# OpenBMB/VisRAG

Hardware: AMD Instinct MI355X
Metric: page-images embedded/sec (VisRAG-Ret encode, 448x448, bf16 MFMA) + queries/sec@top-10 over 100k-page index (higher is better)
Workload: dtype bf16; 1 GPU; VisRAG-Ret (SigLIP-so400m 26 blk + resampler + MiniCPM-2B 40 layers) bf16 encode batch=32 page images 448x448 per GPU; index 100000 rows x 2304 sharded 1 way(s), 1000 queries top-10; batch_per_gpu=32, global_batch=32, parallelism=dp1 (pages sharded, no data-path collective)

## Files before the change

include/visrag_hip.h:

```cpp
#ifndef VISRAG_HIP_H
#define VISRAG_HIP_H

#include <stddef.h>
#include <stdint.h>

#ifdef __cplusplus
extern "C" {
#endif

#define VR_OK 0
#define VR_ERR_INVALID 1
#define VR_ERR_HIP 2
#define VR_ERR_STATE 3
#define VR_ERR_CAPACITY 4

#define VR_DTYPE_F32 0
#define VR_DTYPE_BF16 1

typedef struct vr_model_s* vr_model_t;
typedef struct vr_index_s* vr_index_t;

typedef struct vr_config {
    int32_t patch_size;
    int32_t vit_dim;
// ... 172 lines not shown

int vr_op_gemm(int device_id, const void* A, int32_t lda, const void* W, int32_t ldw,
               int32_t M, int32_t N, int32_t K, int32_t epilogue, const float* bias,
               const float* resid, float alpha, void* out, int32_t ldo,
               const int32_t* rope_pos, const float* rope_table, int32_t rope_cols,
               int32_t variant, void* stream);
typedef struct vr_gemm_extras {
    const int32_t* rowmap;
    const float* rowbias;
    int32_t rowbias_period, rowbias_ld, rowbias_cols;
    float col_scale;
    int32_t col_scale_n;
    int32_t ksplit;
    int64_t split_stride;
    const int32_t* m_dev;
    int32_t m_sub;
    int32_t raster_gm;
} vr_gemm_extras_t;
int vr_op_gemm_ex(int device_id, const void* A, int32_t lda, const void* W, int32_t ldw,
                  int32_t M, int32_t N, int32_t K, int32_t epilogue, const float* bias,
                  const float* resid, float alpha, void* out, int32_t ldo,
                  const int32_t* rope_pos, const float* rope_table, int32_t rope_cols,
                  int32_t variant, const vr_gemm_extras_t* extras, void* stream);
int vr_op_norm(int device_id, int32_t kind, const float* x, int32_t rows, int32_t dim,
               const float* weight, const float* bias, float eps, void* out, int32_t ldo,
               void* stream);
int vr_op_norm_ex(int device_id, int32_t kind, const float* x, int32_t rows, int32_t dim, int32_t ldx, const float* weight,
                  const float* bias, float eps, void* out, int32_t ldo, void* stream);

int vr_op_text_rmsnorm_split(int device_id, const float* x, int32_t rows, int32_t dim, const float* weight, float eps, void* hi,
                             void* lo, void* stream);
int vr_op_text_rope(int device_id, float* qkv, int32_t T, int32_t ld, int32_t rope_cols, const int32_t* pos, const float* table,
                    void* stream);
int vr_op_text_attention(int device_id, const float* qkv, int32_t ld, int32_t E, const int32_t* seq_offsets, int32_t B, int32_t T,
                         int32_t heads, float scale, float* out, void* stream);
int vr_op_text_swiglu_split(int device_id, const float* gu, int32_t T, int32_t ld_gu, int32_t I, int32_t ld_act, void* hi, void* lo,
                            void* stream);
int vr_op_embed_gather(int device_id, const int32_t* ids, int32_t T, const void* table, const void* table_lo, int32_t dim,
                       float scale, float* out, void* stream);
int vr_op_pool(int device_id, const float* h, const int32_t* seq_offsets, int32_t B, int32_t dim, const float* norm_w, float eps,
               float* out, float* tap, int32_t mode, void* stream);
int vr_op_convert(int device_id, int32_t kind, const void* in, void* out, void* out2, int64_t n, int64_t n_total, int32_t* aux,
                  void* stream);
int vr_op_planes_sum(int device_id, const float* parts, int32_t n_parts, int64_t stride, int32_t ldp, int32_t T, int32_t N,
                     float* out, int32_t ldo, float alpha, int32_t accumulate, void* stream);
int vr_op_patch_embed(int device_id, const void* const* imgs, int32_t n, int32_t H, int32_t W, int32_t P, const float* weight,
// ... 45 lines not shown
```

visrag_amd/_lib.py:

```python
from __future__ import annotations

import ctypes as C
import os
from typing import Optional

_HERE = os.path.dirname(os.path.abspath(__file__))
LIB_PATH = os.path.join(_HERE, "libvisrag_hip.so")

VR_DTYPE_F32, VR_DTYPE_BF16 = 0, 1


class VRConfig(C.Structure):
    _fields_ = [
        ("patch_size", C.c_int32), ("vit_dim", C.c_int32), ("vit_depth", C.c_int32),
        ("vit_heads", C.c_int32), ("vit_hidden", C.c_int32), ("vit_pos_grid", C.c_int32),
        ("vit_ln_eps", C.c_float), ("query_num", C.c_int32), ("resampler_ln_eps", C.c_float),
        ("hidden_size", C.c_int32), ("num_layers", C.c_int32), ("num_heads", C.c_int32),
        ("intermediate_size", C.c_int32), ("vocab_size", C.c_int32), ("rms_norm_eps", C.c_float),
        ("rope_theta", C.c_float), ("scale_emb", C.c_float), ("residual_scale", C.c_float),
        ("max_images", C.c_int32), ("max_patches", C.c_int32), ("max_tokens", C.c_int32),
        ("max_seqs", C.c_int32), ("text_split_precision", C.c_int32),
    ]


# ... 73 lines not shown
    "vr_index_search_keys": (C.c_int, [_vp, _vp, _i32, _i32, _i64, _vp, _i32, _vp]),
    "vr_index_set_groups": (C.c_int, [_vp, C.POINTER(_i64), _i64]),
    "vr_index_search_groups": (C.c_int, [_vp, _vp, _i32, _i32, _vp, _vp, _vp, _i32, _vp]),
    "vr_index_group_search_stats": (C.c_int, [_vp, C.POINTER(_i64), _i32]),
    "vr_index_set_filters": (C.c_int, [_vp, _vp, _i32, _i32, _vp]),
    "vr_index_search_filtered": (C.c_int, [_vp, _vp, _i32, _i32, _vp, _vp, _vp, _i32, _vp]),
    "vr_index_filter_search_stats": (C.c_int, [_vp, C.POINTER(_i64), _i32]),
    "vr_index_search_range": (C.c_int, [_vp, _vp, _i32, _vp, _vp, _i64, _vp, C.POINTER(_i64), _i32, _vp]),
    "vr_index_range_results": (C.c_int, [_vp, _vp, _vp, _i64, _i32, _vp]),
    "vr_index_range_search_stats": (C.c_int, [_vp, C.POINTER(_i64), _i32]),
    "vr_index_rank_rows": (C.c_int, [_vp, _vp, _i32, _vp, _vp, _vp, _vp, _vp, _i32, _vp]),
    "vr_index_count_range": (C.c_int, [_vp, _vp, _i32, _vp, _vp, _i32, _vp, _vp, _i32, _vp]),
    "vr_index_rank_search_stats": (C.c_int, [_vp, C.POINTER(_i64), _i32]),
    "vr_index_search_diverse": (C.c_int, [_vp, _vp, _i32, _i32, _i32, _f32, _vp, _vp, _vp, _i32, _vp]),
    "vr_index_remove": (C.c_int, [_vp, C.POINTER(_i64), _i64, C.POINTER(_i64), _vp]),
    "vr_index_update": (C.c_int, [_vp, C.POINTER(_i64), _vp, _i64, _i32, _vp]),
    "vr_index_get_rows": (C.c_int, [_vp, C.POINTER(_i64), _i64, _vp, _vp, _i32, _vp]),
    "vr_topk_merge_keys": (C.c_int, [C.c_int, _vp, _i32, _i32, _i32, _vp, _vp, _vp]),
    "vr_resize_bicubic": (C.c_int, [C.c_int, _vp, _i32, _i32, _i32, _vp, _i32, _i32, _vp]),
    "vr_op_gemm": (C.c_int, [C.c_int, _vp, _i32, _vp, _i32, _i32, _i32, _i32, _i32, _vp, _vp, _f32,
                             _vp, _i32, _vp, _vp, _i32, _i32, _vp]),
    "vr_op_gemm_ex": (C.c_int, [C.c_int, _vp, _i32, _vp, _i32, _i32, _i32, _i32, _i32, _vp, _vp, _f32,
                                _vp, _i32, _vp, _vp, _i32, _i32, C.POINTER(VRGemmExtras), _vp]),
    "vr_op_norm": (C.c_int, [C.c_int, _i32, _vp, _i32, _i32, _vp, _vp, _f32, _vp, _i32, _vp]),
    "vr_op_norm_ex": (C.c_int, [C.c_int, _i32, _vp, _i32, _i32, _i32, _vp, _vp, _f32, _vp, _i32, _vp]),
    "vr_op_text_rmsnorm_split": (C.c_int, [C.c_int, _vp, _i32, _i32, _vp, _f32, _vp, _vp, _vp]),
    "vr_op_text_rope": (C.c_int, [C.c_int, _vp, _i32, _i32, _i32, _vp, _vp, _vp]),
    "vr_op_text_attention": (C.c_int, [C.c_int, _vp, _i32, _i32, _vp, _i32, _i32, _i32, _f32, _vp, _vp]),
    "vr_op_text_swiglu_split": (C.c_int, [C.c_int, _vp, _i32, _i32, _i32, _i32, _vp, _vp, _vp]),
    "vr_op_embed_gather": (C.c_int, [C.c_int, _vp, _i32, _vp, _vp, _i32, _f32, _vp, _vp]),
    "vr_op_pool": (C.c_int, [C.c_int, _vp, _vp, _i32, _i32, _vp, _f32, _vp, _vp, _i32, _vp]),
    "vr_op_convert": (C.c_int, [C.c_int, _i32, _vp, _vp, _vp, _i64, _i64, _vp, _vp]),
    "vr_op_planes_sum": (C.c_int, [C.c_int, _vp, _i32, _i64, _i32, _i32, _i32, _vp, _i32, _f32, _i32, _vp]),
    "vr_op_patch_embed": (C.c_int, [C.c_int, C.POINTER(_vp), _i32, _i32, _i32, _i32, _vp, _i32, _i32, _vp, _vp, _i32, _vp, _i32, _vp]),
    "vr_op_attention": (C.c_int, [C.c_int, _vp, _i32, _vp, _i32, _vp, _i32, _vp, _i32, _vp, _vp, _i32,
                                  _i32, _i32, _i32, _i32, _i32, _f32, _vp]),
    "vr_op_attention_ex": (C.c_int, [C.c_int, _vp, _i32, _vp, _i32, _vp, _i32, _vp, _i32, _vp, _vp, _i32,
                                     _i32, _i32, _i32, _i32, _i32, _f32, C.POINTER(VRAttnExtras), _vp]),
    "vr_op_attn_combine": (C.c_int, [C.c_int, _vp, _vp, _i32, _vp, _i32, _i32, _i32, _vp, _i32, _vp, _i32, _i32, _i32, _i32, _i32,
                                     _i32, _i32, _i64, _vp]),
    "vr_op_gemm_skinny": (C.c_int, [C.c_int, _vp, _i32, _vp, _i32, _i32, _i32, _i32, _i32, _vp, _i32, _vp, _i32, _i64, _vp]),
    "vr_op_plane_sum": (C.c_int, [C.c_int, _i32, _vp, _i32, _i64, _i32, _i32, _i32, _vp, _i32, _f32, _vp, _f32, _vp, _i32, _vp]),
    "vr_op_chat_attention": (C.c_int, [C.c_int, _vp, _vp, _vp, _i32, _i32, _i32, _i32, _i32, _i32, _i32, _i32, C.POINTER(_i32),
                                       C.POINTER(_i32), C.POINTER(_i32), C.POINTER(_i32), _i32, _vp, _vp]),
    "vr_op_chat_select": (C.c_int, [C.c_int, _i32, _vp, _i32, _i32, _vp, _i32, _i32, C.POINTER(_i32), C.POINTER(_f32), _i32, _i32,
                                    _f32, _f32, C.c_uint64, _i32, C.POINTER(_f32), C.POINTER(_i32), C.POINTER(_i32), _vp]),
# ... 77 lines not shown
```

visrag_amd/csrc/encode.hip:

```cpp
#include <hip/hip_runtime.h>

#include <algorithm>
#include <cmath>
#include <cstring>
#include <vector>

#include "model.h"

static int run_vision_group(vr_model_s* m, const uint8_t* const* dev_imgs_hostarray, int n, int H, int W,
                            const int32_t* rowmap_host , bool first_group, hipStream_t s) {
    const vr_config_t& c = m->c;
    const int P = c.patch_size, gh = H / P, gw = W / P, N = gh * gw;
    const int D = m->D, Dp = m->Dp, E = m->E, Q = m->Q;
    const int M = n * N;
    GridTables* g = nullptr;
    VRCHK(get_grid(m, gh, gw, &g));

    HIPCHK(hipMemcpyAsync(m->w_imgptr.p, dev_imgs_hostarray, (size_t)n * 8, hipMemcpyHostToDevice, s));
    int* cu = (int*)arena_take(m, (size_t)2 * (n + 1) * 4);
    for (int i = 0; i <= n; ++i) { cu[i] = i * N; cu[n + 1 + i] = i * Q; }
    HIPCHK(hipMemcpyAsync(m->w_cu.p, cu, (size_t)2 * (n + 1) * 4, hipMemcpyHostToDevice, s));
    HIPCHK(hipMemcpyAsync(m->w_rowmap.p, rowmap_host, (size_t)n * Q * 4, hipMemcpyHostToDevice, s));
    const int* cu_tok = m->w_cu.as<int>();
    const int* cu_qry = m->w_cu.as<int>() + (n + 1);
// ... 335 lines not shown
        }
        if (ks > 1) {
            GemmArgs a = gemm_args(A, lda, L, T, part, E);
            a.ksplit = ks; a.split_stride = pstride;
            HIPCHK(launch_gemm(a, EPI_F32, gemm256w_fits(a, route.proj_variant == GEMM_VARIANT_192W ? 192 : 256) ? route.proj_variant : GEMM_VARIANT_256IL, s));
            pend = true;
        } else {
            GemmArgs a = gemm_args(A, lda, L, T, h, E); a.resid = h; a.alpha = c.residual_scale;
            HIPCHK(launch_gemm(a, EPI_RESID, GEMM_VARIANT_AUTO, s));
        }
        return VR_OK;
    };
    auto norm = [&](const float* w) -> int {
        VRCHK(prof_begin(m, VR_PROF_DEC_NORM, s));
        struct End { vr_model_s* m; hipStream_t s; ~End() { (void)prof_end(m, VR_PROF_DEC_NORM, 0.0, s); } } end_{m, s};
        if (pend) {
            HIPCHK(launch_rmsnorm_accum(h, T, E, E, part, ks, pstride, E, c.residual_scale, w, c.rms_norm_eps, m->w_dxn.p, E, s));
            pend = false;
        } else {
            HIPCHK(launch_rmsnorm(h, T, E, E, w, c.rms_norm_eps, m->w_dxn.p, E, s));
        }
        return VR_OK;
    };
    double attn_flops = 0;
    for (int i = 0; i < B; ++i) { const double Li = seq_offsets[i + 1] - seq_offsets[i]; attn_flops += 4.0 * Li * Li * E; }
    for (int l = 0; l < c.num_layers; ++l) {
        const DecLayer& L = m->layers[l];
        VRCHK(norm(L.ln1.v.as<float>()));
        {
            GemmArgs a = gemm_args(m->w_dxn.p, E, L.qkv, T, m->w_dqkv.p, 3 * E);
            a.rope_pos = m->w_pos.as<int>(); a.rope_table = m->rope.as<float>(); a.rope_cols = 2 * E;
            VRCHK(prof_begin(m, VR_PROF_DEC_QKV, s));
            HIPCHK(launch_gemm(a, EPI_ROPE, GEMM_VARIANT_AUTO, s));
            VRCHK(prof_end(m, VR_PROF_DEC_QKV, 6.0 * T * (double)E * E, s));
        }
        if (hook && hook->layer) VRCHK(hook->layer(hook->ctx, l, m->w_dqkv.p, 3 * E, T, s));
        {
            VRCHK(prof_begin(m, VR_PROF_DEC_ATTN, s));
            AttnArgs a{};
            a.q = m->w_dqkv.p; a.ldq = 3 * E; a.k = (const char*)m->w_dqkv.p + (size_t)E * 2; a.ldk = 3 * E;
            a.v = (const char*)m->w_dqkv.p + (size_t)2 * E * 2; a.ldv = 3 * E;
            a.out = m->w_datt.p; a.ldo = E; a.cu_q = seq; a.cu_kv = seq; a.B = B; a.heads = c.num_heads; a.head_dim = 64;
            a.max_q = max_len; a.causal = 1; a.q_shared = 0; a.scale = 1.0f / sqrtf(64.0f);
            HIPCHK(launch_attention(a, s));
            VRCHK(prof_end(m, VR_PROF_DEC_ATTN, attn_flops, s));
        }
        VRCHK(prof_begin(m, VR_PROF_DEC_O, s));
        VRCHK(proj(m->w_datt.p, E, L.o));
        VRCHK(prof_end(m, VR_PROF_DEC_O, 2.0 * T * (double)E * E, s));
        VRCHK(norm(L.ln2.v.as<float>()));
        VRCHK(prof_begin(m, VR_PROF_DEC_GU, s));
        {
            GemmArgs a = gemm_args(m->w_dxn.p, E, L.gu, T, m->w_dact.p, m->Ip);
            HIPCHK(launch_gemm(a, EPI_SWIGLU, GEMM_VARIANT_AUTO, s));
        }
        VRCHK(prof_end(m, VR_PROF_DEC_GU, 4.0 * T * (double)E * m->I, s));
        VRCHK(prof_begin(m, VR_PROF_DEC_DOWN, s));
        VRCHK(proj(m->w_dact.p, m->Ip, L.down));
        VRCHK(prof_end(m, VR_PROF_DEC_DOWN, 2.0 * T * (double)E * m->I, s));
        if (l == 0) VRCHK(tap_store(m, "dec_layer0", h, T, E, E, false, s));
    }
    if (pend) {
        HIPCHK(launch_rmsnorm_accum(h, T, E, E, part, ks, pstride, E, c.residual_scale, nullptr, c.rms_norm_eps, nullptr, 0, s));
        pend = false;
    }
    }
    {
        double fl = 0;
        for (int i = 0; i < B; ++i) { const double Li = seq_offsets[i + 1] - seq_offsets[i]; fl += 4.0 * Li * Li * E; }
        fl = c.num_layers * (fl + (double)T * (8.0 * E * E + 6.0 * (double)E * m->I));
        VRCHK(prof_end(m, VR_PROF_DECODER, fl, s));
    }
    float* tap_hidden = nullptr;
    if (m->taps_on && (size_t)T * E * 4 <= m->w_kv32.bytes) tap_hidden = m->w_kv32.as<float>();
    if (out_hidden) {
        if (max_len > hidden_len) return fail(VR_ERR_INVALID, "hidden_len=%d is shorter than the longest sequence (%d)", hidden_len, max_len);
// ... 19 lines not shown
```

visrag_amd/csrc/gemm.hip:

```cpp
#include "gemm_core.h"
#include "gemm_core_il.h"
#include "kernels.h"
#include "gemm_epilogue.h"

namespace vr {

template <int EPI>
__global__ __launch_bounds__(256) void gemm_bf16_kernel(GemmArgs p) {
    extern __shared__ __attribute__((aligned(16))) char smem[];
    const int tiles_n = p.N / GEMM_BN;
    const int tiles_m = (p.M + GEMM_BM - 1) / GEMM_BM;
    const int t = xcd_remap(blockIdx.x, tiles_m * tiles_n);
    const int GM = p.raster_gm > 0 ? p.raster_gm : 1;
    const int gsz = GM * tiles_n;
    const int g = t / gsz, r = t % gsz;
    const int gm = min(GM, tiles_m - g * GM);
    const int m0 = (g * GM + r % gm) * GEMM_BM, n0 = (r / gm) * GEMM_BN;

    gemm_acc_t acc;
    gemm_zero(acc);
    gemm_mainloop(acc, (const bf16_t*)p.A, p.lda, (const bf16_t*)p.W, p.ldw, m0, n0, p.K, smem);

    const int lane = threadIdx.x & 63, wave = threadIdx.x >> 6;
    const int wm = wave >> 1, wn = wave & 1;
// ... 78 lines not shown
        return hipGetLastError();
    }
    if (variant != GEMM_VARIANT_GLDS) return hipErrorInvalidValue;
    const int tiles = (a.N / GEMM_BN) * ((a.M + GEMM_BM - 1) / GEMM_BM);
    if (a.raster_gm <= 0) {
        const int tm = (a.M + GEMM_BM - 1) / GEMM_BM;
        a.raster_gm = tm <= 32 ? tm : 4;
    }
    auto k = gemm_bf16_kernel<EPI>;
    static unsigned long long attr = 0;
    set_max_dynamic_lds((const void*)k, GEMM_SMEM_BYTES, attr);
    hipLaunchKernelGGL(k, dim3(tiles), dim3(256), GEMM_SMEM_BYTES, s, a);
    return hipGetLastError();
}

bool gemm_args_refused(const GemmArgs& a, int epi, int variant) {
    if (a.col_scale_n != 0 && (epi != EPI_BF16 || a.col_scale_n < 0 || a.col_scale_n % 64 != 0)) return true;
    const bool half_tile = variant == GEMM_VARIANT_128W_192 || variant == GEMM_VARIANT_128W_256;
    const bool split_tile = variant == GEMM_VARIANT_256IL || variant == GEMM_VARIANT_256W || variant == GEMM_VARIANT_192W;
    if (half_tile && (a.rowmap || a.rowbias)) return true;
    if (a.rowbias && ((epi != EPI_BF16 && epi != EPI_GELU && epi != EPI_F32) || a.rowbias_period < 1)) return true;
    if (a.ksplit > 1 && (!split_tile || epi != EPI_F32 || a.K % (a.ksplit * GEMM_BK) || a.rowmap || a.rowbias)) return true;
    if (a.m_dev && variant != GEMM_VARIANT_256IL) return true;
    return false;
}

hipError_t launch_gemm(const GemmArgs& a, int epi, int variant, hipStream_t s) {
    if (a.M <= 0) return hipSuccess;
    if (variant == GEMM_VARIANT_192) return launch_gemm192(a, epi, s);
    if (variant == GEMM_VARIANT_256W) return launch_gemm256w(a, epi, s);
    if (variant == GEMM_VARIANT_192W) return launch_gemm192w(a, epi, s);
    if (variant == GEMM_VARIANT_128W_192) return launch_gemm128w(a, epi, 192, s);
    if (variant == GEMM_VARIANT_128W_256) return launch_gemm128w(a, epi, 256, s);
    if (variant == GEMM_VARIANT_AUTO) {
        if (a.N % 192 == 0 && a.N % 256 != 0 && a.N <= 1536 && a.M >= 4096 && epi <= EPI_RESID) {
            if (epi == EPI_RESID && !a.rowmap && gemm256w_fits(a, 192)) return launch_gemm192w(a, epi, s);
            return launch_gemm192(a, epi, s);
        }
        const bool n_ok = (a.N % 256 == 0) || a.N >= 2048;
        const long t256 = (long)((a.N + 255) / 256) * ((a.M + 255) / 256);
        const long t128 = (long)(a.N / 128) * ((a.M + 127) / 128);
        const double e256 = 1.45 * (double)t256 / (double)(((t256 + 255) / 256) * 256);
        const double e128 = (double)t128 / (double)(((t128 + 511) / 512) * 512);
        const bool w_ok = gemm256w_fits(a, 256);
        variant = (n_ok && e256 > e128) ? (w_ok ? GEMM_VARIANT_256W : GEMM_VARIANT_256IL) : GEMM_VARIANT_GLDS;
        if (variant == GEMM_VARIANT_256W) return launch_gemm256w(a, epi, s);
    }
    if (gemm_args_refused(a, epi, variant)) return hipErrorInvalidValue;
    switch (epi) {
        case EPI_BF16: return launch_epi<EPI_BF16>(a, variant, s);
        case EPI_GELU: return launch_epi<EPI_GELU>(a, variant, s);
        case EPI_F32: return launch_epi<EPI_F32>(a, variant, s);
        case EPI_RESID: return launch_epi<EPI_RESID>(a, variant, s);
        case EPI_SWIGLU: return launch_epi<EPI_SWIGLU>(a, variant, s);
        case EPI_ROPE: return launch_epi<EPI_ROPE>(a, variant, s);
        default: return hipErrorInvalidValue;
    }
}

}
```

visrag_amd/csrc/gemm256w.hip:

```cpp
#include <type_traits>

#include "gemm_core.h"
#include "gemm_epilogue.h"
#include "gemm256w_acc.h"

namespace vr {

bool gemm256w_fits(const GemmArgs& a, int bn);

namespace {

constexpr int W_STAGE = 2 * G256_TILE_BYTES;
constexpr unsigned W_OOB = 0x80000000u;

}

constexpr int W_STAGING = 4096;
constexpr int W_SMEM_BYTES = 2 * W_STAGE + 4 * W_STAGING;

#define W_KERNEL_TEMPLATE template <int EPI, bool PLAIN, int NJ>
#define W_KERNEL_NAME gemm256w_bf16_kernel
#include "gemm256w_kernel.h"
#undef W_KERNEL_TEMPLATE
#undef W_KERNEL_NAME

template <int EPI, bool PLAIN, int NJ>
static hipError_t launch_wp(GemmArgs a, hipStream_t s) {
    constexpr int BN = 32 * NJ;
    const int tn = (a.N + BN - 1) / BN, tm = (a.M + G256_BM - 1) / G256_BM;
    if (a.raster_gm <= 0) a.raster_gm = tm <= 16 ? tm : 4;
    if (!gemm256w_fits(a, BN)) return hipErrorInvalidValue;
    if (gemm_args_refused(a, EPI, NJ == 6 ? GEMM_VARIANT_192W : GEMM_VARIANT_256W)) return hipErrorInvalidValue;
    int total = tn * tm;
    if (a.ksplit > 1) total *= a.ksplit;
    auto k = gemm256w_bf16_kernel<EPI, PLAIN, NJ>;
    static unsigned long long attr = 0;
    set_max_dynamic_lds((const void*)k, W_SMEM_BYTES, attr);
    hipLaunchKernelGGL(k, dim3(total), dim3(256), W_SMEM_BYTES, s, a);
    return hipGetLastError();
}

// ... 37 lines not shown
```

visrag_amd/csrc/gemm256w_kernel.h:

```cpp
W_KERNEL_TEMPLATE
__global__ __launch_bounds__(256) __attribute__((amdgpu_waves_per_eu(1, 1))) void W_KERNEL_NAME(GemmArgs p) {
    static_assert(NJ == 8 || (NJ == 6 && !PLAIN), "wave tile 128 x 128 or 128 x 96");
    constexpr int BN = 32 * NJ;
    constexpr int NS = 8 * NJ;
    constexpr int NR = 8 + NJ;
    constexpr int DS = NJ == 8 ? 5 : 4;
    constexpr int SB1 = NS * 5 / 8;
    constexpr int D1 = (NS - 1 - (SB1 + 2)) / DS + 1;
    constexpr int SB2 = NJ;
    constexpr int NF = NJ / 2;
    static_assert(SB2 + 3 + DS * (NR - D1 - 1) < NS && SB2 + 2 + 2 * (NR - 1) < NS && 2 * NR - 2 < SB1, "schedule fits");
    extern __shared__ __attribute__((aligned(16))) char smem[];
#ifdef VR_W_TIMING
    const unsigned long long tm0 = __builtin_amdgcn_s_memrealtime();
    unsigned long long tm1 = 0, tm2 = 0, cy1 = 0, cy2 = 0;
#endif
    const int tiles_n = (p.N + BN - 1) / BN;
    const int tiles_m = (p.M + G256_BM - 1) / G256_BM;
    const int ks = p.ksplit > 1 ? p.ksplit : 1;
    const int total = tiles_m * tiles_n * ks;
    const int Ks = p.K / ks;
    const int nk = Ks / GEMM_BK;

    const int my_first = xcd_remap(blockIdx.x, total);
// ... 25 lines not shown
    auto tile_off_w = [&](int n0, int split) { return ((unsigned)n0 * (unsigned)p.ldw + (unsigned)split * (unsigned)Ks) * 2u; };

    auto dma = [&](int stage, int d, unsigned vA, unsigned vW) {
        if (d < 8) __builtin_amdgcn_raw_ptr_buffer_load_lds(arsrc, VR_LDS(dmaA + stage * W_STAGE + d * 1024), 16, vA, sA0 + d * rgA, 0, 0);
        else __builtin_amdgcn_raw_ptr_buffer_load_lds(wrsrc, VR_LDS(dmaW + stage * W_STAGE + (d - 8) * 1024), 16, vW, sW0 + (d - 8) * rgW, 0, 0);
    };

    typedef const __attribute__((address_space(3))) bf16x8* frag_p;
    frag_p pA[2][2], pW[2][2];
#pragma unroll
    for (int st = 0; st < 2; ++st)
#pragma unroll
        for (int kk = 0; kk < 2; ++kk) {
            const int ch = ((kk * 4 + fq) ^ (fr & 7)) << 4;
            pA[st][kk] = (frag_p)VR_LDS(smem + st * W_STAGE + (wm * 128 + fr) * 128 + ch);
            pW[st][kk] = (frag_p)VR_LDS(smem + st * W_STAGE + G256_TILE_BYTES + (wn * 16 * NJ + fr) * 128 + ch);
            asm volatile("" : "+v"(pA[st][kk]), "+v"(pW[st][kk]));
        }

    bf16x8 a0[8], w0[NJ], a1[8], w1[NJ];
    int m0, n0, split;
    coords(my_first, m0, n0, split);
    unsigned curA = tile_off_a(m0, split), curW = tile_off_w(n0, split);

    {
        const unsigned k1 = nk > 1 ? (unsigned)(GEMM_BK * 2) : W_OOB;
#pragma unroll
        for (int d = 0; d < NR; ++d) dma(0, d, lofA + curA, lofW + curW);
#pragma unroll
        for (int d = 0; d < NR; ++d) dma(1, d, lofA + curA + k1, lofW + curW + k1);
        W_FOR_EACH_ACC(W_ZERO)
        if constexpr (NJ == 8) VR_WAIT_VM_BARRIER(16); else VR_WAIT_VM_BARRIER(14);
#pragma unroll
        for (int j = 0; j < NJ; ++j) w0[j] = pW[0][0][j * 128];
#pragma unroll
        for (int i = 0; i < 8; ++i) a0[i] = pA[0][0][i * 128];
    }
#ifdef VR_W_TIMING
    asm volatile("s_waitcnt lgkmcnt(0)" ::: "memory");
    tm1 = __builtin_amdgcn_s_memrealtime();
    cy1 = __builtin_amdgcn_s_memtime();
#endif

    {
        const unsigned nxtA = W_OOB, nxtW = W_OOB;

        auto step = [&](auto stage_c, int kt) {
            constexpr int S = decltype(stage_c)::value;
            const int k2 = kt + 2;
            const unsigned vA = lofA + (k2 < nk ? curA + (unsigned)k2 * (GEMM_BK * 2) : nxtA + (unsigned)(k2 - nk) * (GEMM_BK * 2));
            const unsigned vW = lofW + (k2 < nk ? curW + (unsigned)k2 * (GEMM_BK * 2) : nxtW + (unsigned)(k2 - nk) * (GEMM_BK * 2));
            __builtin_amdgcn_sched_barrier(0);
            auto aux1 = [&](int sl) {
// ... 26 lines not shown
#undef W_P1
#undef W_P2
        };

        for (int kt = 0; kt < nk; kt += 2) {
            step(std::integral_constant<int, 0>{}, kt);
            if (kt + 1 >= nk) break;
            step(std::integral_constant<int, 1>{}, kt + 1);
        }
        asm volatile("s_nop 15\n\ts_nop 15" ::: "memory");
#ifdef VR_W_TIMING
        tm2 = __builtin_amdgcn_s_memrealtime();
        cy2 = __builtin_amdgcn_s_memtime();
#endif

        const int mrow0 = m0 + wm * 128, nb0 = n0 + wn * (16 * NJ);
        char* const wl0 = smem + 2 * W_STAGE + wave * W_STAGING;
        bool plain_resid = false;
        if constexpr (EPI == EPI_RESID) plain_resid = !p.rowmap;
        auto uni32 = [](unsigned v) { return (unsigned)__builtin_amdgcn_readfirstlane((int)v); };
        auto uni_ptr = [&](const void* q) {
            const unsigned long long a = (unsigned long long)q;
            return (void*)(((unsigned long long)uni32((unsigned)(a >> 32)) << 32) | uni32((unsigned)a));
        };
        bool buf_tile = false;
        if constexpr (EPI == EPI_RESID) buf_tile = plain_resid && n0 + BN <= p.N;
        if constexpr (EPI == EPI_F32) buf_tile = !p.rowmap && !p.rowbias && n0 + BN <= p.N;
        if constexpr (EPI == EPI_RESID || EPI == EPI_F32) {
            if (buf_tile) {
                constexpr int MI = 2;
                const float alpha = __builtin_bit_cast(float, uni32(__builtin_bit_cast(unsigned, p.alpha)));
                const unsigned ldb = uni32((unsigned)p.ldo * 4u);
                const unsigned nrec = uni32((unsigned)min(G256_BM, p.M - m0) * ldb);
                float* obase = (float*)p.out + (size_t)m0 * p.ldo;
                if constexpr (EPI == EPI_F32) obase += (size_t)split * p.split_stride;
                const auto ors = __builtin_amdgcn_make_buffer_rsrc(uni_ptr(obase), 0, nrec, 0x00020000);
                const bool with_bias = p.bias && (EPI == EPI_RESID || split == 0);
                const auto brs = __builtin_amdgcn_make_buffer_rsrc(uni_ptr(p.bias), 0, uni32(with_bias ? (unsigned)p.N * 4u : 0u), 0x00020000);
                const unsigned voff = (unsigned)(wm * 128 + fr) * ldb + (unsigned)(nb0 + fq * 4) * 4u;
                f32x4 bias[NJ];
#pragma unroll
                for (int j = 0; j < NJ; ++j)
                    bias[j] = __builtin_bit_cast(f32x4, __builtin_amdgcn_raw_buffer_load_b128(brs, (unsigned)(nb0 + fq * 4) * 4u + j * 64, 0, 0));
                if constexpr (EPI == EPI_RESID) {
                    constexpr int RD = NJ == 6 ? 3 : 2;
                    const auto rrs = __builtin_amdgcn_make_buffer_rsrc(uni_ptr(p.resid + (size_t)m0 * p.ldo), 0, nrec, 0x00020000);
                    f32x4 rs[RD + 1][MI][NF];
                    auto load_piece = [&](int q, f32x4 (&dst)[MI][NF]) {
                        const int h = q & 1, sg = q >> 1;
#pragma unroll
                        for (int i = 0; i < MI; ++i)
#pragma unroll
                            for (int j = 0; j < NF; ++j)
                                dst[i][j] = __builtin_bit_cast(f32x4, __builtin_amdgcn_raw_buffer_load_b128(
                                    rrs, voff + (unsigned)((sg * MI + i) * 16) * ldb + (h * NF + j) * 64, 0, 0));
                    };
#pragma unroll
                    for (int q = 0; q < RD; ++q) load_piece(q, rs[q]);
#pragma unroll
                    for (int q = 0; q < 8; ++q) {
                        const int h = q & 1, sg = q >> 1;
                        if (q + RD < 8) load_piece(q + RD, rs[(q + RD) % (RD + 1)]);
                        f32x4 acc[MI][NF];
#define W_RD(n, R, C0, C1, C2, C3) \
                        if (((n) & 7) < NJ && ((n) & 7) / NF == h && ((n) >> 4) == sg) W_READ(acc[((n) >> 3) & 1][((n) & 7) % NF], C0, C1, C2, C3);
                        W_FOR_EACH_ACC(W_RD)
#undef W_RD
#pragma unroll
                        for (int i = 0; i < MI; ++i)
#pragma unroll
                            for (int j = 0; j < NF; ++j) {
                                const f32x4 v = rs[q % (RD + 1)][i][j] + alpha * (acc[i][j] + bias[h * NF + j]);
                                __builtin_amdgcn_raw_buffer_store_b128(__builtin_bit_cast(u32x4, v), ors,
                                                                       voff + (unsigned)((sg * MI + i) * 16) * ldb + (h * NF + j) * 64, 0, 0);
                            }
                        __builtin_amdgcn_sched_barrier(0);
                    }
                } else {
#pragma unroll
                    for (int q = 0; q < 8; ++q) {
                        const int h = q & 1, sg = q >> 1;
                        f32x4 acc[MI][NF];
#define W_RD(n, R, C0, C1, C2, C3) \
                        if (((n) & 7) < NJ && ((n) & 7) / NF == h && ((n) >> 4) == sg) W_READ(acc[((n) >> 3) & 1][((n) & 7) % NF], C0, C1, C2, C3);
                        W_FOR_EACH_ACC(W_RD)
#undef W_RD
#pragma unroll
                        for (int i = 0; i < MI; ++i)
#pragma unroll
                            for (int j = 0; j < NF; ++j)
                                __builtin_amdgcn_raw_buffer_store_b128(__builtin_bit_cast(u32x4, acc[i][j] + bias[h * NF + j]), ors,
                                                                       voff + (unsigned)((sg * MI + i) * 16) * ldb + (h * NF + j) * 64, 0, 0);
                        __builtin_amdgcn_sched_barrier(0);
                    }
                }
            }
        }
        if constexpr (EPI == EPI_RESID) {
            if (plain_resid && !buf_tile) {
                constexpr int MI = 2;
                const float* __restrict__ resid = p.resid;
                float* __restrict__ out = (float*)p.out;
                constexpr int RD = 1;
                f32x4 rs[RD + 1][MI][NF];
                auto load_piece = [&](int q, f32x4 (&dst)[MI][NF]) {
                    const int h = q & 1, sg = q >> 1;
#pragma unroll
                    for (int i = 0; i < MI; ++i) {
                        const size_t ro = (size_t)min(mrow0 + (sg * MI + i) * 16 + fr, p.M - 1) * p.ldo;
#pragma unroll
                        for (int j = 0; j < NF; ++j) {
                            dst[i][j] = *reinterpret_cast<const f32x4*>(resid + ro + min(nb0 + (h * NF + j) * 16 + fq * 4, p.N - 4));
                        }
                    }
                };
#pragma unroll
                for (int q = 0; q < RD; ++q) load_piece(q, rs[q]);
                f32x4 bias[NJ];
#pragma unroll
                for (int j = 0; j < NJ; ++j)
                    bias[j] = p.bias ? *reinterpret_cast<const f32x4*>(p.bias + min(nb0 + j * 16 + fq * 4, p.N - 4)) : f32x4{0.f, 0.f, 0.f, 0.f};
#pragma unroll
                for (int q = 0; q < 8; ++q) {
                    const int h = q & 1, sg = q >> 1;
                    if (q + RD < 8) load_piece(q + RD, rs[(q + RD) % (RD + 1)]);
                    f32x4 acc[MI][NF];
#define W_RD(n, R, C0, C1, C2, C3) \
                    if (((n) & 7) < NJ && ((n) & 7) / NF == h && ((n) >> 4) == sg) W_READ(acc[((n) >> 3) & 1][((n) & 7) % NF], C0, C1, C2, C3);
                    W_FOR_EACH_ACC(W_RD)
#undef W_RD
#pragma unroll
                    for (int i = 0; i < MI; ++i) {
                        const int m = mrow0 + (sg * MI + i) * 16 + fr;
#pragma unroll
                        for (int j = 0; j < NF; ++j) {
                            const int n = nb0 + (h * NF + j) * 16 + fq * 4;
                            if (m < p.M && n < p.N)
                                *reinterpret_cast<f32x4*>(out + (size_t)m * p.ldo + n) = rs[q % (RD + 1)][i][j] + p.alpha * (acc[i][j] + bias[h * NF + j]);
                        }
                    }
                    __builtin_amdgcn_sched_barrier(0);
                }
            }
        }
// ... 10 lines not shown
            }
            const bool rb_on = EPI == EPI_BF16 && PLAIN && p.rowbias != nullptr;
            const auto rbrs = __builtin_amdgcn_make_buffer_rsrc(uni_ptr(p.rowbias), 0,
                                                                uni32(rb_on ? (unsigned)p.rowbias_period * (unsigned)p.rowbias_ld * 4u : 0u), 0x00020000);
            const unsigned rb_row0 = rb_on ? uni32((unsigned)(m0 % p.rowbias_period)) : 0u;
            int posw[8];
#pragma unroll
            for (int t = 0; t < 8; ++t) posw[t] = 0;
            if constexpr (EPI == EPI_ROPE && PLAIN) {
#pragma unroll
                for (int t = 0; t < 8; ++t) posw[t] = p.rope_pos[min(mrow0 + t * 16 + fr, p.M - 1)];
            }
            f32x4 rt[2][2][4];
            auto load_rope = [&](int sg, f32x4 (&d)[2][4]) {
#pragma unroll
                for (int i = 0; i < 2; ++i) {
                    const float* tab = p.rope_table + (size_t)posw[sg * 2 + i] * 64 + fq * 4;
#pragma unroll
                    for (int j = 0; j < 4; ++j) d[i][j] = *reinterpret_cast<const f32x4*>(tab + j * 16);
                }
            };
            if constexpr (EPI == EPI_ROPE && PLAIN) load_rope(0, rt[0]);
            (void)ors16; (void)ldo2; (void)biasw; (void)rbrs; (void)rb_row0; (void)posw; (void)rt;
#pragma unroll
            for (int q = 0; q < 8; ++q) {
                constexpr int MI = 2;
                const int h = q & 1, sg = q >> 1;
                f32x4 acc[MI][NF];
#define W_RD(n, R, C0, C1, C2, C3) \
                if (((n) & 7) < NJ && ((n) & 7) / NF == h && ((n) >> 4) == sg) W_READ(acc[((n) >> 3) & 1][((n) & 7) % NF], C0, C1, C2, C3);
                W_FOR_EACH_ACC(W_RD)
#undef W_RD
                const int mr = mrow0 + sg * 32, nb = nb0 + h * (16 * NF);
                bool done = false;
                if constexpr (EPI == EPI_F32) {
                    if (!p.rowmap && !p.rowbias) {
                        float* __restrict__ out = (float*)p.out + (size_t)split * p.split_stride;
                        const float* bp = split == 0 ? p.bias : nullptr;
                        f32x4 bias[NF];
#pragma unroll
                        for (int j = 0; j < NF; ++j)
                            bias[j] = bp ? *reinterpret_cast<const f32x4*>(bp + min(nb + j * 16 + fq * 4, p.N - 4)) : f32x4{0.f, 0.f, 0.f, 0.f};
#pragma unroll
                        for (int i = 0; i < MI; ++i) {
                            const int m = mr + i * 16 + fr;
#pragma unroll
// ... 58 lines not shown
```

visrag_amd/csrc/kernels.h:

```cpp
#pragma once
#include <hip/hip_runtime.h>
#include <stdint.h>

namespace vr {

enum GemmEpilogue { EPI_BF16 = 0, EPI_GELU = 1, EPI_F32 = 2, EPI_RESID = 3, EPI_SWIGLU = 4, EPI_ROPE = 5 };
enum GemmVariant { GEMM_VARIANT_GLDS = 0, GEMM_VARIANT_AUTO = 3, GEMM_VARIANT_192 = 7, GEMM_VARIANT_256IL = 9, GEMM_VARIANT_256W = 12,
                   GEMM_VARIANT_192W = 13, GEMM_VARIANT_128W_192 = 14, GEMM_VARIANT_128W_256 = 15 };

struct GemmArgs {
    const void* A; int lda;
    const void* W; int ldw;
    int M, N, K;
    const float* bias;
    const float* resid;
    float alpha;
    void* out; int ldo;
    const int* rowmap;
    const float* rowbias;
    int rowbias_period, rowbias_ld, rowbias_cols;
    const int* rope_pos;
    const float* rope_table;
    int rope_cols;
    int raster_gm;
    int ksplit;
    size_t split_stride;
    float col_scale; int col_scale_n;
    const int* m_dev; int m_sub;
};
hipError_t launch_gemm(const GemmArgs& a, int epilogue, int variant, hipStream_t s);
bool gemm_args_refused(const GemmArgs& a, int epilogue, int variant);
hipError_t launch_gemm192(const GemmArgs& a, int epilogue, hipStream_t s);
hipError_t launch_gemm256w(const GemmArgs& a, int epilogue, hipStream_t s);
bool gemm256w_fits(const GemmArgs& a, int tile_cols);
hipError_t launch_gemm192w(const GemmArgs& a, int epilogue, hipStream_t s);
hipError_t launch_gemm128w(const GemmArgs& a, int epilogue, int tile_cols, hipStream_t s);
bool gemm128w_fits(const GemmArgs& a, int tile_cols);

struct SkinnyCombine { const void* part; const float* lse; int S; int heads; int group; const int* S_dev; };
hipError_t launch_gemm_skinny(const GemmArgs& a, hipStream_t s, bool swiglu = false, const struct SkinnyCombine* combine = nullptr);
hipError_t launch_swiglu_sum(const float* parts, int n_parts, size_t plane_stride, int ldp, int M, int I, void* act, int lda,
                             hipStream_t s);

hipError_t launch_layernorm(const float* x, int rows, int dim, int ldx, const float* w, const float* b,
                            float eps, void* out, int ldo, hipStream_t s);
hipError_t launch_rmsnorm_accum(float* x, int rows, int dim, int ldx, const float* partial, int nsplit,
                                size_t split_stride, int ldp, float alpha, const float* w, float eps, void* out,
                                int ldo, hipStream_t s);
hipError_t launch_rmsnorm(const float* x, int rows, int dim, int ldx, const float* w, float eps,
                          void* out, int ldo, hipStream_t s);

struct AttnArgs {
    const void* q; int ldq;
    const void* k; int ldk;
// ... 276 lines not shown
```

visrag_amd/csrc/ops.hip:

```cpp
#include <hip/hip_runtime.h>

#include <algorithm>
#include <chrono>
#include <map>
#include <tuple>
#include <vector>

#include "engine_common.h"

struct ResizeTab { DevBuf bounds, kk; int ksize = 0; };
static std::map<std::tuple<int, int, int>, ResizeTab> g_resize_tabs;

static int get_resize_tab(int dev, int in_size, int out_size, ResizeTab** out) {
    auto key = std::make_tuple(dev, in_size, out_size);
    auto it = g_resize_tabs.find(key);
    if (it == g_resize_tabs.end()) {
        std::vector<int> b, k;
        ResizeTab t;
        t.ksize = resize_coeffs(in_size, out_size, b, k);
        VRCHK(t.bounds.alloc(b.size() * 4));
        VRCHK(t.kk.alloc(k.size() * 4));
        HIPCHK(hipMemcpy(t.bounds.p, b.data(), b.size() * 4, hipMemcpyHostToDevice));
        HIPCHK(hipMemcpy(t.kk.p, k.data(), k.size() * 4, hipMemcpyHostToDevice));
        it = g_resize_tabs.emplace(key, std::move(t)).first;
// ... 54 lines not shown

extern "C" int vr_streams_overlap(int device_id, void* stream_a, void* stream_b, int32_t* overlap) {
    if (!overlap) return fail(VR_ERR_INVALID, "NULL argument");
    VRCHK(set_dev(device_id));
    const hipStream_t a = (hipStream_t)stream_a, b = (hipStream_t)stream_b;
    constexpr int usec = 400;
    int votes = 0;
    for (int rep = 0; rep < 3; ++rep) {
        HIPCHK(hipStreamSynchronize(a));
        HIPCHK(hipStreamSynchronize(b));
        const auto t0 = std::chrono::steady_clock::now();
        hipLaunchKernelGGL(spin_kernel, dim3(1), dim3(1), 0, a, (long long)usec * 100);
        hipLaunchKernelGGL(spin_kernel, dim3(1), dim3(1), 0, b, (long long)usec * 100);
        HIPCHK(hipGetLastError());
        HIPCHK(hipStreamSynchronize(a));
        HIPCHK(hipStreamSynchronize(b));
        const double us = std::chrono::duration<double, std::micro>(std::chrono::steady_clock::now() - t0).count();
        if (rep > 0) votes += us < 1.6 * usec ? 1 : 0;
    }
    *overlap = votes == 2 ? 1 : 0;
    return VR_OK;
}

extern "C" int vr_op_gemm_ex(int device_id, const void* A, int32_t lda, const void* W, int32_t ldw, int32_t M, int32_t N,
                             int32_t K, int32_t epilogue, const float* bias, const float* resid, float alpha, void* out,
                             int32_t ldo, const int32_t* rope_pos, const float* rope_table, int32_t rope_cols,
                             int32_t variant, const vr_gemm_extras_t* extras, void* stream) {
    if (!A || !W || !out) return fail(VR_ERR_INVALID, "NULL argument");
    if (variant != GEMM_VARIANT_GLDS && variant != GEMM_VARIANT_AUTO && variant != GEMM_VARIANT_192 && variant != GEMM_VARIANT_256IL && variant != GEMM_VARIANT_256W && variant != GEMM_VARIANT_192W &&
        variant != GEMM_VARIANT_128W_192 && variant != GEMM_VARIANT_128W_256)
        return fail(VR_ERR_INVALID, "variant %d: 0 (128^2 tile), 3 (auto), 7 (256x192 tile), 9 (256^2 tile), 12 / 13 (256^2 / 256x192 tile, one wave per SIMD), 14 / 15 (128x192 / 128x256 tile, one wave per SIMD)", variant);
    if (((variant == 7 || variant == 13 || variant == 14) ? N % 192 : N % 128) || K % 64 || M <= 0) return fail(VR_ERR_INVALID, "need N %% 128 == 0 (192 for variant 7), K %% 64 == 0");
    if (epilogue == EPI_RESID && !resid) return fail(VR_ERR_INVALID, "EPI_RESID needs resid");
    if (epilogue == EPI_ROPE && (!rope_pos || !rope_table)) return fail(VR_ERR_INVALID, "EPI_ROPE needs tables");
    VRCHK(set_dev(device_id));
    GemmArgs a{};
    a.A = A; a.lda = lda; a.W = W; a.ldw = ldw; a.M = M; a.N = N; a.K = K; a.bias = bias; a.resid = resid;
    a.alpha = alpha; a.out = out; a.ldo = ldo; a.rope_pos = rope_pos; a.rope_table = rope_table; a.rope_cols = rope_cols;
    if (extras) {
        a.rowmap = extras->rowmap;
        a.rowbias = extras->rowbias; a.rowbias_period = extras->rowbias_period; a.rowbias_ld = extras->rowbias_ld; a.rowbias_cols = extras->rowbias_cols;
        a.col_scale = extras->col_scale; a.col_scale_n = extras->col_scale_n;
        a.ksplit = extras->ksplit; a.split_stride = (size_t)extras->split_stride;
        a.m_dev = extras->m_dev; a.m_sub = extras->m_sub;
        a.raster_gm = extras->raster_gm;
    }
    HIPCHK(launch_gemm(a, epilogue, variant, (hipStream_t)stream));
    return VR_OK;
}

extern "C" int vr_op_gemm(int device_id, const void* A, int32_t lda, const void* W, int32_t ldw, int32_t M, int32_t N,
                          int32_t K, int32_t epilogue, const float* bias, const float* resid, float alpha, void* out,
                          int32_t ldo, const int32_t* rope_pos, const float* rope_table, int32_t rope_cols,
                          int32_t variant, void* stream) {
    return vr_op_gemm_ex(device_id, A, lda, W, ldw, M, N, K, epilogue, bias, resid, alpha, out, ldo, rope_pos, rope_table, rope_cols,
                         variant, nullptr, stream);
}

extern "C" int vr_op_norm(int device_id, int32_t kind, const float* x, int32_t rows, int32_t dim, const float* weight,
                          const float* bias, float eps, void* out, int32_t ldo, void* stream) {
    if (!x || !weight || !out || (kind == 0 && !bias)) return fail(VR_ERR_INVALID, "NULL argument");
    VRCHK(set_dev(device_id));
    if (kind == 0) HIPCHK(launch_layernorm(x, rows, dim, dim, weight, bias, eps, out, ldo, (hipStream_t)stream));
    else HIPCHK(launch_rmsnorm(x, rows, dim, dim, weight, eps, out, ldo, (hipStream_t)stream));
    return VR_OK;
}

extern "C" int vr_op_attention_ex(int device_id, const void* q, int32_t ldq, const void* k, int32_t ldk, const void* v,
                                  int32_t ldv, void* out, int32_t ldo, const int32_t* cu_q, const int32_t* cu_kv, int32_t B,
                                  int32_t heads, int32_t head_dim, int32_t max_q, int32_t causal, int32_t q_shared,
                                  float scale, const vr_attn_extras_t* extras, void* stream) {
// ... 322 lines not shown
```

Before: 717.2 pages/s.

## Prefetch next decoder GEMM weights into cache during the 256W GEMM epilogue

Adds a 'warm' region to the 256W GEMM kernel. Each wave issues buffer loads (dumped into a small LDS scratch) that pull the next layer's weight matrix (W_o after QKV, W_down after gate/up) into cache while the current GEMM runs its epilogue. The goal is to hide the cold HBM fetch of the following GEMM's weights behind the current kernel's tail. In exchange it spends extra memory bandwidth, some LDS, and extra instructions in the epilogue. The auto-variant choice is moved into a reusable function so the host can tell whether the 256W kernel will be used.

```diff
diff --git a/include/visrag_hip.h b/include/visrag_hip.h
--- a/include/visrag_hip.h
+++ b/include/visrag_hip.h
@@ -218,6 +218,11 @@
                   const float* resid, float alpha, void* out, int32_t ldo,
                   const int32_t* rope_pos, const float* rope_table, int32_t rope_cols,
                   int32_t variant, const vr_gemm_extras_t* extras, void* stream);
+int vr_op_gemm_warm(int device_id, const void* A, int32_t lda, const void* W, int32_t ldw,
+                    int32_t M, int32_t N, int32_t K, int32_t epilogue, const float* bias,
+                    const float* resid, float alpha, void* out, int32_t ldo,
+                    const int32_t* rope_pos, const float* rope_table, int32_t rope_cols,
+                    int32_t variant, const vr_gemm_extras_t* extras, const void* warm, uint64_t warm_bytes, void* stream);
 int vr_op_norm(int device_id, int32_t kind, const float* x, int32_t rows, int32_t dim,
                const float* weight, const float* bias, float eps, void* out, int32_t ldo,
                void* stream);
diff --git a/visrag_amd/_lib.py b/visrag_amd/_lib.py
--- a/visrag_amd/_lib.py
+++ b/visrag_amd/_lib.py
@@ -119,6 +119,8 @@
                              _vp, _i32, _vp, _vp, _i32, _i32, _vp]),
     "vr_op_gemm_ex": (C.c_int, [C.c_int, _vp, _i32, _vp, _i32, _i32, _i32, _i32, _i32, _vp, _vp, _f32,
                                 _vp, _i32, _vp, _vp, _i32, _i32, C.POINTER(VRGemmExtras), _vp]),
+    "vr_op_gemm_warm": (C.c_int, [C.c_int, _vp, _i32, _vp, _i32, _i32, _i32, _i32, _i32, _vp, _vp, _f32,
+                                  _vp, _i32, _vp, _vp, _i32, _i32, C.POINTER(VRGemmExtras), _vp, C.c_uint64, _vp]),
     "vr_op_norm": (C.c_int, [C.c_int, _i32, _vp, _i32, _i32, _vp, _vp, _f32, _vp, _i32, _vp]),
     "vr_op_norm_ex": (C.c_int, [C.c_int, _i32, _vp, _i32, _i32, _i32, _vp, _vp, _f32, _vp, _i32, _vp]),
     "vr_op_text_rmsnorm_split": (C.c_int, [C.c_int, _vp, _i32, _i32, _vp, _f32, _vp, _vp, _vp]),
diff --git a/visrag_amd/csrc/encode.hip b/visrag_amd/csrc/encode.hip
--- a/visrag_amd/csrc/encode.hip
+++ b/visrag_amd/csrc/encode.hip
@@ -381,6 +381,10 @@
         }
         return VR_OK;
     };
+    auto warm_for = [&](GemmArgs& a, int epi, const Linear& next) {
+        const size_t bytes = (size_t)next.n_pad * next.k_pad * 2;
+        if (route.proj_128w && !hook && bytes < WARM_MAX_BYTES && gemm_auto_variant(a, epi) == GEMM_VARIANT_256W) { a.warm = next.w.p; a.warm_bytes = bytes; }
+    };
     double attn_flops = 0;
     for (int i = 0; i < B; ++i) { const double Li = seq_offsets[i + 1] - seq_offsets[i]; attn_flops += 4.0 * Li * Li * E; }
     for (int l = 0; l < c.num_layers; ++l) {
@@ -389,6 +393,7 @@
         {
             GemmArgs a = gemm_args(m->w_dxn.p, E, L.qkv, T, m->w_dqkv.p, 3 * E);
             a.rope_pos = m->w_pos.as<int>(); a.rope_table = m->rope.as<float>(); a.rope_cols = 2 * E;
+            warm_for(a, EPI_ROPE, L.o);
             VRCHK(prof_begin(m, VR_PROF_DEC_QKV, s));
             HIPCHK(launch_gemm(a, EPI_ROPE, GEMM_VARIANT_AUTO, s));
             VRCHK(prof_end(m, VR_PROF_DEC_QKV, 6.0 * T * (double)E * E, s));
@@ -411,6 +416,7 @@
         VRCHK(prof_begin(m, VR_PROF_DEC_GU, s));
         {
             GemmArgs a = gemm_args(m->w_dxn.p, E, L.gu, T, m->w_dact.p, m->Ip);
+            warm_for(a, EPI_SWIGLU, L.down);
             HIPCHK(launch_gemm(a, EPI_SWIGLU, GEMM_VARIANT_AUTO, s));
         }
         VRCHK(prof_end(m, VR_PROF_DEC_GU, 4.0 * T * (double)E * m->I, s));
diff --git a/visrag_amd/csrc/gemm.hip b/visrag_amd/csrc/gemm.hip
--- a/visrag_amd/csrc/gemm.hip
+++ b/visrag_amd/csrc/gemm.hip
@@ -124,30 +124,32 @@
     if (a.rowbias && ((epi != EPI_BF16 && epi != EPI_GELU && epi != EPI_F32) || a.rowbias_period < 1)) return true;
     if (a.ksplit > 1 && (!split_tile || epi != EPI_F32 || a.K % (a.ksplit * GEMM_BK) || a.rowmap || a.rowbias)) return true;
     if (a.m_dev && variant != GEMM_VARIANT_256IL) return true;
+    if (a.warm && a.warm_bytes && (variant != GEMM_VARIANT_256W || a.warm_bytes >= WARM_MAX_BYTES)) return true;
     return false;
+}
+
+int gemm_auto_variant(const GemmArgs& a, int epi) {
+    if (a.N % 192 == 0 && a.N % 256 != 0 && a.N <= 1536 && a.M >= 4096 && epi <= EPI_RESID) {
+        if (epi == EPI_RESID && !a.rowmap && gemm256w_fits(a, 192)) return GEMM_VARIANT_192W;
+        return GEMM_VARIANT_192;
+    }
+    const bool n_ok = (a.N % 256 == 0) || a.N >= 2048;
+    const long t256 = (long)((a.N + 255) / 256) * ((a.M + 255) / 256);
+    const long t128 = (long)(a.N / 128) * ((a.M + 127) / 128);
+    const double e256 = 1.45 * (double)t256 / (double)(((t256 + 255) / 256) * 256);
+    const double e128 = (double)t128 / (double)(((t128 + 511) / 512) * 512);
+    const bool w_ok = gemm256w_fits(a, 256);
+    return (n_ok && e256 > e128) ? (w_ok ? GEMM_VARIANT_256W : GEMM_VARIANT_256IL) : GEMM_VARIANT_GLDS;
 }
 
 hipError_t launch_gemm(const GemmArgs& a, int epi, int variant, hipStream_t s) {
     if (a.M <= 0) return hipSuccess;
+    if (variant == GEMM_VARIANT_AUTO) variant = gemm_auto_variant(a, epi);
     if (variant == GEMM_VARIANT_192) return launch_gemm192(a, epi, s);
     if (variant == GEMM_VARIANT_256W) return launch_gemm256w(a, epi, s);
     if (variant == GEMM_VARIANT_192W) return launch_gemm192w(a, epi, s);
     if (variant == GEMM_VARIANT_128W_192) return launch_gemm128w(a, epi, 192, s);
     if (variant == GEMM_VARIANT_128W_256) return launch_gemm128w(a, epi, 256, s);
-    if (variant == GEMM_VARIANT_AUTO) {
-        if (a.N % 192 == 0 && a.N % 256 != 0 && a.N <= 1536 && a.M >= 4096 && epi <= EPI_RESID) {
-            if (epi == EPI_RESID && !a.rowmap && gemm256w_fits(a, 192)) return launch_gemm192w(a, epi, s);
-            return launch_gemm192(a, epi, s);
-        }
-        const bool n_ok = (a.N % 256 == 0) || a.N >= 2048;
-        const long t256 = (long)((a.N + 255) / 256) * ((a.M + 255) / 256);
-        const long t128 = (long)(a.N / 128) * ((a.M + 127) / 128);
-        const double e256 = 1.45 * (double)t256 / (double)(((t256 + 255) / 256) * 256);
-        const double e128 = (double)t128 / (double)(((t128 + 511) / 512) * 512);
-        const bool w_ok = gemm256w_fits(a, 256);
-        variant = (n_ok && e256 > e128) ? (w_ok ? GEMM_VARIANT_256W : GEMM_VARIANT_256IL) : GEMM_VARIANT_GLDS;
-        if (variant == GEMM_VARIANT_256W) return launch_gemm256w(a, epi, s);
-    }
     if (gemm_args_refused(a, epi, variant)) return hipErrorInvalidValue;
     switch (epi) {
         case EPI_BF16: return launch_epi<EPI_BF16>(a, variant, s);
diff --git a/visrag_amd/csrc/gemm256w.hip b/visrag_amd/csrc/gemm256w.hip
--- a/visrag_amd/csrc/gemm256w.hip
+++ b/visrag_amd/csrc/gemm256w.hip
@@ -16,7 +16,35 @@
 }
 
 constexpr int W_STAGING = 4096;
-constexpr int W_SMEM_BYTES = 2 * W_STAGE + 4 * W_STAGING;
+constexpr int W_WARM_DUMP = 256;
+constexpr int W_SMEM_BYTES = 2 * W_STAGE + 4 * W_STAGING + 4 * W_WARM_DUMP;
+
+constexpr bool warm_shares_tile(size_t bytes, unsigned total) {
+    unsigned at = 0;
+    for (unsigned w = 0; w < total; ++w)
+        for (unsigned v = 0; v < WARM_WAVES; ++v) {
+            const WarmShare s = warm_share(bytes, w, total, v);
+            if (s.first != at || s.end < s.first) return false;
+            at = s.end;
+        }
+    return at == warm_lines(bytes) && (size_t)at * WARM_LINE >= bytes && (bytes == 0 || (size_t)(at - 1) * WARM_LINE < bytes);
+}
+static_assert(warm_shares_tile(0, 1) && warm_shares_tile(0, 243), "no lines");
+static_assert(warm_shares_tile(1, 1) && warm_shares_tile(WARM_LINE, 4) && warm_shares_tile(WARM_LINE + 1, 4), "1 and 2 lines");
+static_assert(warm_shares_tile(63 * WARM_LINE, 1) && warm_shares_tile(64 * WARM_LINE, 1) && warm_shares_tile(65 * WARM_LINE, 1), "63 / 64 / 65 lines, one workgroup");
+static_assert(warm_shares_tile(63 * WARM_LINE, 4) && warm_shares_tile(64 * WARM_LINE, 4) && warm_shares_tile(65 * WARM_LINE - 3, 4), "63 / 64 / 65 lines, four");
+static_assert(warm_shares_tile(100 * WARM_LINE, 243) && warm_shares_tile(5 * WARM_LINE, 405), "a region of fewer lines than the grid has waves");
+static_assert(warm_shares_tile((size_t)2304 * 2304 * 2, 243), "W_o (10.6 MB) over the decoder's q|k|v grid");
+static_assert(warm_shares_tile((size_t)2304 * 5760 * 2, 405), "W_down (26.5 MB) over the decoder's gate|up grid");
+static_assert(warm_shares_tile(WARM_MAX_BYTES - 1, 1021), "the largest region");
+static_assert(warm_cut((1u << 24) - 1, 65534, 65535) == (unsigned)(((1ull << 24) - 1) * 65534 / 65535) && warm_cut(65534, 65534, 65535) == 65533 &&
+              warm_cut((1u << 24) - 1, 65535, 65535) == (1u << 24) - 1, "the largest grid of the 32-bit form");
+static_assert(warm_part(0, warm_lines(WARM_MAX_BYTES - 1), 65536, 65537).end == warm_lines(WARM_MAX_BYTES - 1) &&
+              warm_cut(1u << 24, 70001, 70003) == (unsigned)((1ull << 24) * 70001 / 70003) && warm_cut(82944, 100, 243) == 82944ull * 100 / 243, "both forms of the cut");
+#if VR_WARM_LINE == 128
+static_assert(warm_instructions(warm_share((size_t)2304 * 2304 * 2, 0, 243, 0)) == 2 &&
+              warm_instructions(warm_share((size_t)2304 * 5760 * 2, 404, 405, 3)) == 2, "two requests per wave in the decoder");
+#endif
 
 #define W_KERNEL_TEMPLATE template <int EPI, bool PLAIN, int NJ>
 #define W_KERNEL_NAME gemm256w_bf16_kernel
diff --git a/visrag_amd/csrc/gemm256w_kernel.h b/visrag_amd/csrc/gemm256w_kernel.h
--- a/visrag_amd/csrc/gemm256w_kernel.h
+++ b/visrag_amd/csrc/gemm256w_kernel.h
@@ -71,6 +71,7 @@
     int m0, n0, split;
     coords(my_first, m0, n0, split);
     unsigned curA = tile_off_a(m0, split), curW = tile_off_w(n0, split);
+    unsigned warm_lo = 0, warm_hi = 0;
 
     {
         const unsigned k1 = nk > 1 ? (unsigned)(GEMM_BK * 2) : W_OOB;
@@ -78,6 +79,13 @@
         for (int d = 0; d < NR; ++d) dma(0, d, lofA + curA, lofW + curW);
 #pragma unroll
         for (int d = 0; d < NR; ++d) dma(1, d, lofA + curA + k1, lofW + curW + k1);
+        if constexpr (NJ == 8) {
+            if (p.warm && p.warm_bytes) {
+                const WarmShare sh = warm_share(p.warm_bytes, (unsigned)my_first, (unsigned)total, (unsigned)wave);
+                warm_lo = (unsigned)__builtin_amdgcn_readfirstlane((int)sh.first);
+                warm_hi = (unsigned)__builtin_amdgcn_readfirstlane((int)sh.end);
+            }
+        }
         W_FOR_EACH_ACC(W_ZERO)
         if constexpr (NJ == 8) VR_WAIT_VM_BARRIER(16); else VR_WAIT_VM_BARRIER(14);
 #pragma unroll
@@ -150,6 +158,26 @@
         auto uni_ptr = [&](const void* q) {
             const unsigned long long a = (unsigned long long)q;
             return (void*)(((unsigned long long)uni32((unsigned)(a >> 32)) << 32) | uni32((unsigned)a));
+        };
+        auto warm_requests = [&]() {
+            if constexpr (NJ == 8) {
+                if (warm_lo < warm_hi) {
+                    const unsigned long long wa = (unsigned long long)uni_ptr(p.warm);
+                    const auto wrs = __builtin_amdgcn_make_buffer_rsrc((void*)wa, 0, uni32((unsigned)p.warm_bytes), 0x00020000);
+                    const unsigned pad = (0u - (unsigned)wa) & 3u;
+                    char* const dump = smem + 2 * W_STAGE + 4 * W_STAGING + wave * W_WARM_DUMP;
+                    auto request = [&](unsigned l) {
+                        const unsigned line = l + (unsigned)lane;
+                        __builtin_amdgcn_raw_ptr_buffer_load_lds(wrs, VR_LDS(dump), 4, line < warm_hi ? line * WARM_LINE + pad : W_OOB, 0, 0, 0);
+                    };
+                    __builtin_amdgcn_sched_barrier(0);
+                    request(warm_lo);
+                    request(warm_lo + 64);
+                    __builtin_amdgcn_sched_barrier(0);
+#pragma nounroll
+                    for (unsigned l = warm_lo + 128; l < warm_hi; l += 64) request(l);
+                }
+            }
         };
         bool buf_tile = false;
         if constexpr (EPI == EPI_RESID) buf_tile = plain_resid && n0 + BN <= p.N;
@@ -185,6 +213,7 @@
                     };
 #pragma unroll
                     for (int q = 0; q < RD; ++q) load_piece(q, rs[q]);
+                    warm_requests();
 #pragma unroll
                     for (int q = 0; q < 8; ++q) {
                         const int h = q & 1, sg = q >> 1;
@@ -205,6 +234,7 @@
                         __builtin_amdgcn_sched_barrier(0);
                     }
                 } else {
+                    warm_requests();
 #pragma unroll
                     for (int q = 0; q < 8; ++q) {
                         const int h = q & 1, sg = q >> 1;
@@ -248,6 +278,7 @@
 #pragma unroll
                 for (int j = 0; j < NJ; ++j)
                     bias[j] = p.bias ? *reinterpret_cast<const f32x4*>(p.bias + min(nb0 + j * 16 + fq * 4, p.N - 4)) : f32x4{0.f, 0.f, 0.f, 0.f};
+                warm_requests();
 #pragma unroll
                 for (int q = 0; q < 8; ++q) {
                     const int h = q & 1, sg = q >> 1;
@@ -304,6 +335,7 @@
             };
             if constexpr (EPI == EPI_ROPE && PLAIN) load_rope(0, rt[0]);
             (void)ors16; (void)ldo2; (void)biasw; (void)rbrs; (void)rb_row0; (void)posw; (void)rt;
+            warm_requests();
 #pragma unroll
             for (int q = 0; q < 8; ++q) {
                 constexpr int MI = 2;
diff --git a/visrag_amd/csrc/gemm_warm.h b/visrag_amd/csrc/gemm_warm.h
--- /dev/null
+++ b/visrag_amd/csrc/gemm_warm.h
@@ -0,0 +1,31 @@
+#pragma once
+#include <hip/hip_runtime.h>
+#include <stddef.h>
+
+namespace vr {
+
+#ifndef VR_WARM_LINE
+#define VR_WARM_LINE 128
+#endif
+constexpr unsigned WARM_LINE = VR_WARM_LINE;
+constexpr unsigned WARM_WAVES = 4;
+constexpr size_t WARM_MAX_BYTES = (size_t)1 << 31;
+
+struct WarmShare { unsigned first, end; };
+
+__host__ __device__ constexpr unsigned warm_lines(size_t bytes) { return (unsigned)((bytes + WARM_LINE - 1) / WARM_LINE); }
+
+__host__ __device__ constexpr unsigned warm_cut(unsigned n, unsigned w, unsigned total) {
+    if (total < 65536u) return n / total * w + n % total * w / total;
+    return (unsigned)((unsigned long long)n * w / total);
+}
+__host__ __device__ constexpr WarmShare warm_part(unsigned lo, unsigned hi, unsigned w, unsigned total) {
+    return WarmShare{lo + warm_cut(hi - lo, w, total), lo + warm_cut(hi - lo, w + 1, total)};
+}
+__host__ __device__ constexpr WarmShare warm_share(size_t bytes, unsigned w, unsigned total, unsigned wave) {
+    const WarmShare g = warm_part(0, warm_lines(bytes), w, total);
+    return warm_part(g.first, g.end, wave, WARM_WAVES);
+}
+__host__ __device__ constexpr unsigned warm_instructions(WarmShare s) { return (s.end - s.first + 63) / 64; }
+
+}
diff --git a/visrag_amd/csrc/kernels.h b/visrag_amd/csrc/kernels.h
--- a/visrag_amd/csrc/kernels.h
+++ b/visrag_amd/csrc/kernels.h
@@ -1,6 +1,8 @@
 #pragma once
 #include <hip/hip_runtime.h>
 #include <stdint.h>
+
+#include "gemm_warm.h"
 
 namespace vr {
 
@@ -27,9 +29,11 @@
     size_t split_stride;
     float col_scale; int col_scale_n;
     const int* m_dev; int m_sub;
+    const void* warm; size_t warm_bytes;
 };
 hipError_t launch_gemm(const GemmArgs& a, int epilogue, int variant, hipStream_t s);
 bool gemm_args_refused(const GemmArgs& a, int epilogue, int variant);
+int gemm_auto_variant(const GemmArgs& a, int epilogue);
 hipError_t launch_gemm192(const GemmArgs& a, int epilogue, hipStream_t s);
 hipError_t launch_gemm256w(const GemmArgs& a, int epilogue, hipStream_t s);
 bool gemm256w_fits(const GemmArgs& a, int tile_cols);
diff --git a/visrag_amd/csrc/ops.hip b/visrag_amd/csrc/ops.hip
--- a/visrag_amd/csrc/ops.hip
+++ b/visrag_amd/csrc/ops.hip
@@ -100,10 +100,10 @@
     return VR_OK;
 }
 
-extern "C" int vr_op_gemm_ex(int device_id, const void* A, int32_t lda, const void* W, int32_t ldw, int32_t M, int32_t N,
-                             int32_t K, int32_t epilogue, const float* bias, const float* resid, float alpha, void* out,
-                             int32_t ldo, const int32_t* rope_pos, const float* rope_table, int32_t rope_cols,
-                             int32_t variant, const vr_gemm_extras_t* extras, void* stream) {
+extern "C" int vr_op_gemm_warm(int device_id, const void* A, int32_t lda, const void* W, int32_t ldw, int32_t M, int32_t N,
+                               int32_t K, int32_t epilogue, const float* bias, const float* resid, float alpha, void* out,
+                               int32_t ldo, const int32_t* rope_pos, const float* rope_table, int32_t rope_cols,
+                               int32_t variant, const vr_gemm_extras_t* extras, const void* warm, uint64_t warm_bytes, void* stream) {
     if (!A || !W || !out) return fail(VR_ERR_INVALID, "NULL argument");
     if (variant != GEMM_VARIANT_GLDS && variant != GEMM_VARIANT_AUTO && variant != GEMM_VARIANT_192 && variant != GEMM_VARIANT_256IL && variant != GEMM_VARIANT_256W && variant != GEMM_VARIANT_192W &&
         variant != GEMM_VARIANT_128W_192 && variant != GEMM_VARIANT_128W_256)
@@ -123,8 +123,17 @@
         a.m_dev = extras->m_dev; a.m_sub = extras->m_sub;
         a.raster_gm = extras->raster_gm;
     }
+    a.warm = warm; a.warm_bytes = (size_t)warm_bytes;
     HIPCHK(launch_gemm(a, epilogue, variant, (hipStream_t)stream));
     return VR_OK;
+}
+
+extern "C" int vr_op_gemm_ex(int device_id, const void* A, int32_t lda, const void* W, int32_t ldw, int32_t M, int32_t N,
+                             int32_t K, int32_t epilogue, const float* bias, const float* resid, float alpha, void* out,
+                             int32_t ldo, const int32_t* rope_pos, const float* rope_table, int32_t rope_cols,
+                             int32_t variant, const vr_gemm_extras_t* extras, void* stream) {
+    return vr_op_gemm_warm(device_id, A, lda, W, ldw, M, N, K, epilogue, bias, resid, alpha, out, ldo, rope_pos, rope_table, rope_cols,
+                           variant, extras, nullptr, 0, stream);
 }
 
 extern "C" int vr_op_gemm(int device_id, const void* A, int32_t lda, const void* W, int32_t ldw, int32_t M, int32_t N,
```

After: 728.4 pages/s (median of 6 runs). 1.02x the previous value.
